# wenbowen123/iros20-6d-pose-tracking

Hardware: NVIDIA H100
Metric: rgbd_pair_frames_per_sec (higher is better)
Workload: dtype bf16x3 (bf16 hi/lo split operands, 3 products/MAC, fp32 accumulate)

## Files before the change

iros20-6d-pose-tracking_b200/csrc/conv_common.h:

```cpp
#pragma once
#include <cstdint>
#include <cuda.h>
#include <cuda_runtime.h>

namespace se3tn {

constexpr int kMaxTaps = 9;
constexpr int kBlockM = 128;
constexpr int kChunkBytes = 128;

enum Act : int { ACT_NONE = 0, ACT_RELU = 1, ACT_SELU = 2 };
enum { KIND_S1 = 0, KIND_S2 = 1, KIND_STEM = 2 };

struct Tap {
    int16_t dy, dx;
};

struct ConvGeom {
    int Hin, Win, in_cstride, in_coff;
    int Ho, Wo, stride;
    int cin;
    int cout;
    int groups;
    int num_taps;
// ... 44 lines not shown

constexpr int kTrunkMaxLayers = 6;

struct TrunkParams {
    LayerDesc layer[kTrunkMaxLayers];
    int n_layers;
    int total_units;
    int img_first, n_img;
    int max_batch;
    unsigned* sched;
    const int* img_wid;
    const CUtensorMap* gbmaps;
    const float* const* gbias;
    unsigned long long* trace;
    int ksplit;
    float* partial;
    unsigned* slice_cnt;
};

struct ResidentParams {
    LayerDesc L;
    int img_first, n_img;
    int m_tiles;
    int step_x, step_y, off_x, off_y;
    const int* img_wid;
    const CUtensorMap* gbmaps;
    const float* const* gbias;
    unsigned long long* trace;
};

cudaError_t launch_conv_resident(const ResidentParams& p, int kind, int prec, int num_sms, bool pdl, cudaStream_t stream);
cudaError_t launch_conv_trunk(const TrunkParams& p, int prec, int num_sms, bool pdl, cudaStream_t stream);
constexpr int kSplitMaxImages = 4, kSplitK = 4, kSplitMaxUnits = kSplitMaxImages * 8 * kTrunkMaxLayers;
inline size_t trunk_sched_words(int max_batch) { return 1 + static_cast<size_t>(kTrunkMaxLayers) * max_batch + static_cast<size_t>(kSplitMaxUnits) * 8; }
inline size_t trunk_partial_floats() { return static_cast<size_t>(kSplitMaxUnits) * kSplitK * 128 * 128; }

cudaError_t launch_conv_direct(const ConvGeom& g, const ConvPtrs& p, cudaStream_t stream);

}
```

iros20-6d-pose-tracking_b200/csrc/conv_wgmma.cu:

```cuda
#include "conv_common.h"
#include "ptx.cuh"
#include "storage.cuh"
#include <algorithm>

namespace se3tn {
namespace {

constexpr int kThreads2 = 384;
constexpr int kPoolPitch = 68;
constexpr int kPoolStageBytes = 121 * kPoolPitch * 4;
constexpr int kPoolStageAlloc = (kPoolStageBytes + 1023) & ~1023;
constexpr int kAUnit3 = 19 * 1024;
constexpr int kAUnitStem = 21 * 1024;
constexpr int kWgRowBytes = 64 * kChunkBytes;

template <int KIND> struct KTab;
template <> struct KTab<KIND_S1> {
    static constexpr int NU = 3;
    __host__ __device__ static constexpr int ntaps(int) { return 3; }
    __host__ __device__ static constexpr int wtap(int u, int k) { return k * 3 + u; }
    __host__ __device__ static constexpr int amap(int) { return 0; }
    __host__ __device__ static constexpr int c1(int u) { return u - 1; }
    __host__ __device__ static constexpr int c2(int) { return -1; }
    __host__ __device__ static constexpr int rows(int) { return 11 * 13; }
// ... 300 lines not shown
                    const int pp = v >> 4, c4 = (v & 15) * 4;
                    const int ppy = pp / 5, ppx = pp - ppy * 5;
                    const int oy = ty * 5 + ppy, ox = tx * 5 + ppx;
                    if (oy >= L.Ho || ox >= L.Wo) continue;
                    float4 mx = make_float4(-3.0e38f, -3.0e38f, -3.0e38f, -3.0e38f);
#pragma unroll
                    for (int dy = 0; dy < 3; ++dy)
#pragma unroll
                        for (int dx = 0; dx < 3; ++dx) {
                            const float4 s4 = *reinterpret_cast<const float4*>(stage + ((2 * ppy + dy) * 11 + 2 * ppx + dx) * kPoolPitch + c4);
                            mx.x = fmaxf(mx.x, s4.x); mx.y = fmaxf(mx.y, s4.y); mx.z = fmaxf(mx.z, s4.z); mx.w = fmaxf(mx.w, s4.w);
                        }
                    const float4 b4 = __ldg(reinterpret_cast<const float4*>(bias + c4));
                    const float v4[4] = {selu_fast(mx.x + b4.x), selu_fast(mx.y + b4.y), selu_fast(mx.z + b4.z), selu_fast(mx.w + b4.w)};
                    S::encode(v4).store(L.out + S::addr((static_cast<size_t>(n0) * L.Ho + oy) * L.Wo + ox, L.out_c, L.out_coff + c4));
                }
                if (C::kPoolBufs == 1) asm volatile("bar.sync 1, 256;" ::: "memory");
            }
        }
        if (stamp) { trace_stamp(p.trace, 4); trace_stamp(p.trace, 6); }
    }

    __syncthreads();
    if (threadIdx.x == 0) trace_exit(p.trace);
}

template <int PREC> struct TCfg {
    static constexpr int BN = 128;
    static constexpr int kAcc = BN / 2;
    static constexpr int kAStages = 3;
    static constexpr int kBStages = 6;
    static constexpr int kBTile = BN * kChunkBytes;
    static constexpr int kEpiPitch = 36;
    static constexpr int kEpiWarpBytes = 16 * kEpiPitch * 4 + 64;
    static constexpr int kEpiBytes = 8 * kEpiWarpBytes;
    static constexpr int kSched = 4;
    static constexpr int kSmem = kAStages * kAUnit3 + kBStages * kBTile + ((kEpiBytes + 1023) & ~1023) + 1024 + 512;
    static_assert(kSmem <= 232448, "shared memory budget");
};

struct UnitCoord { int l, img, tx, ty, n_tile, grp, c0, c1, piece, gidx; };
__device__ __forceinline__ void unit_stamp(const TrunkParams& p, int u, int k) {
    if (p.trace && u < 2048) p.trace[256 * 8 + u * 5 + k] = gtimer();
}

__device__ __forceinline__ int unit_layer(const TrunkParams& p, int u) {
    int l = 0;
#pragma unroll
    for (int i = 1; i < kTrunkMaxLayers; ++i) if (i < p.n_layers && u >= p.layer[i].unit_base) l = i;
    return l;
}

__device__ __forceinline__ UnitCoord decode_unit(const TrunkParams& p, int u) {
    UnitCoord c;
    c.l = unit_layer(p, u);
    const LayerDesc& L = p.layer[c.l];
    int local = u - L.unit_base;
    c.piece = 0; c.c0 = 0; c.c1 = L.chunks;
    if (p.ksplit > 1) {
        c.piece = local % p.ksplit; local /= p.ksplit;
        c.c0 = c.piece * L.chunks / p.ksplit; c.c1 = (c.piece + 1) * L.chunks / p.ksplit;
    }
    c.gidx = L.base_unit0 + local;
    const int im = local / L.units_per_image;
    int r = local - im * L.units_per_image;
    c.img = p.img_first + im;
    c.n_tile = r % L.n_tiles; r /= L.n_tiles;
    c.grp = r % L.groups; r /= L.groups;
    c.ty = r / L.tiles_x; c.tx = r - c.ty * L.tiles_x;
    return c;
}

template <int KIND>
__device__ __forceinline__ void trunk_load_unit(const LayerDesc& L, const UnitCoord& c, uint8_t* sA, uint64_t* a_full, uint64_t* a_empty,
                                                int& stage, uint32_t& phase, int n_stages)
{
// ... 3 lines not shown
    for (int ch = c.c0; ch < c.c1; ++ch) {
#pragma unroll
        for (int u = 0; u < KT::NU; ++u) {
            ptx::mbar_wait(&a_empty[stage], phase ^ 1);
            ptx::mbar_arrive_expect_tx(&a_full[stage], static_cast<uint32_t>(KT::rows(u)) * kChunkBytes);
            ptx::tma_load_4d(sA + stage * kAUnit3, &L.amap[KT::amap(u)], &a_full[stage], cbase + ch * 32, ox + KT::c1(u), oy + KT::c2(u), c.img);
            if (++stage == n_stages) { stage = 0; phase ^= 1; }
        }
    }
}

template <int KIND, int PREC>
__device__ __forceinline__ void trunk_load_weights(const LayerDesc& L, const CUtensorMap* bm, const UnitCoord& c, uint8_t* sB,
                                                   uint64_t* b_full, uint64_t* b_empty, int& stage, uint32_t& phase)
{
    using KT = KTab<KIND>;
    using C = TCfg<PREC>;
    const int wrow = c.grp * L.cout + c.n_tile * C::BN;
    for (int ch = c.c0; ch < c.c1; ++ch) {
#pragma unroll
        for (int u = 0; u < KT::NU; ++u) {
#pragma unroll
            for (int k = 0; k < KT::ntaps(u); ++k) {
                ptx::mbar_wait(&b_empty[stage], phase ^ 1);
                ptx::mbar_arrive_expect_tx(&b_full[stage], C::kBTile);
                ptx::tma_load_2d(sB + stage * C::kBTile, bm, &b_full[stage], KT::wtap(u, k) * L.cin_words + ch * 32, wrow);
                if (++stage == C::kBStages) { stage = 0; phase ^= 1; }
            }
        }
    }
}

template <int KIND, int PREC>
__device__ __forceinline__ void trunk_mma_unit(float (&acc)[TCfg<PREC>::kAcc], const Consumer& cs, int chunks, uint8_t* sA, uint8_t* sB,
                                               uint64_t* a_full, uint64_t* a_empty, uint64_t* b_full, uint64_t* b_empty,
                                               int& astage, uint32_t& aphase, int& bstage, uint32_t& bphase,
                                               unsigned long long* trace, bool first_unit, unsigned long long* ustamp)
{
    using KT = KTab<KIND>;
    using C = TCfg<PREC>;
    const bool stamp = threadIdx.x == 128;
    uint32_t fresh = 0;
    int pend_b = -1, pend_a = -1;
    for (int ch = 0; ch < chunks; ++ch) {
#pragma unroll
        for (int u = 0; u < KT::NU; ++u) {
            ptx::mbar_wait(&a_full[astage], aphase);
            if (first_unit && ch == 0 && u == 0 && stamp) trace_stamp(trace, 3);
            if (ustamp && ch == 0 && u == 0 && stamp) *ustamp = gtimer();
            const uint32_t a_unit_lo = desc_lo(sA + astage * kAUnit3 + cs.cg * kWgRowBytes);
#pragma unroll
            for (int k = 0; k < KT::ntaps(u); ++k) {
                ptx::mbar_wait(&b_full[bstage], bphase);
                if (first_unit && ch == 0 && u == 0 && k == 0 && stamp) trace_stamp(trace, 2);
                const uint32_t b_lo = desc_lo(sB + bstage * C::kBTile);
                const uint32_t a_lo = a_unit_lo + k * kRowShift * (kChunkBytes >> 4);
                ptx::wgmma_fence();
                if constexpr (PREC == SE3TN_PREC_TF32) {
#pragma unroll
                    for (int kk = 0; kk < 4; ++kk)
                        ptx::wgmma_tf32_n128(acc, mk_desc(a_lo + 2 * kk), mk_desc(b_lo + 2 * kk), fresh | (kk ? 1u : 0u));
                } else if constexpr (PREC == SE3TN_PREC_BF16X3) {
                    constexpr int AO[6] = {0, 2, 4, 6, 0, 2};
                    constexpr int BO[6] = {0, 2, 0, 2, 4, 6};
#pragma unroll
                    for (int i = 0; i < 6; ++i)
                        ptx::wgmma_bf16_n128(acc, mk_desc(a_lo + AO[i]), mk_desc(b_lo + BO[i]), fresh | (i ? 1u : 0u));
                } else {
#pragma unroll
                    for (int kk = 0; kk < 4; ++kk)
                        ptx::wgmma_bf16_n128(acc, mk_desc(a_lo + 2 * kk), mk_desc(b_lo + 2 * kk), fresh | (kk ? 1u : 0u));
                }
                ptx::wgmma_commit();
                ptx::wgmma_wait<1>();
                if (cs.leader()) {
                    if (pend_b >= 0) ptx::mbar_arrive(&b_empty[pend_b]);
                    if (pend_a >= 0) ptx::mbar_arrive(&a_empty[pend_a]);
                }
                pend_b = bstage;
                pend_a = (k + 1 == KT::ntaps(u)) ? astage : -1;
                fresh = 1u;
                if (++bstage == C::kBStages) { bstage = 0; bphase ^= 1; }
            }
            if (++astage == C::kAStages) { astage = 0; aphase ^= 1; }
        }
    }
    ptx::wgmma_wait<0>();
    ptx::wgmma_reg_fence(acc);
    if (cs.leader()) {
        if (pend_b >= 0) ptx::mbar_arrive(&b_empty[pend_b]);
        if (pend_a >= 0) ptx::mbar_arrive(&a_empty[pend_a]);
    }
}

template <int PREC>
__global__ void __launch_bounds__(kThreads2, 1)
conv_trunk_kernel(const __grid_constant__ TrunkParams p)
{
    using C = TCfg<PREC>;
    constexpr int BN = C::BN;
    extern __shared__ uint8_t smem_raw[];
    uint8_t* smem = reinterpret_cast<uint8_t*>((reinterpret_cast<uintptr_t>(smem_raw) + 1023) & ~uintptr_t(1023));
    uint8_t* sA = smem;
    uint8_t* sB = sA + C::kAStages * kAUnit3;
    uint8_t* sT = sB + C::kBStages * C::kBTile;
    uint64_t* bars = reinterpret_cast<uint64_t*>(sT + ((C::kEpiBytes + 1023) & ~1023));
    uint64_t* a_full = bars;
    uint64_t* a_empty = a_full + C::kAStages;
    uint64_t* b_full = a_empty + C::kAStages;
    uint64_t* b_empty = b_full + C::kBStages;
    uint64_t* sched_full = b_empty + C::kBStages;
    uint64_t* sched_empty = sched_full + C::kSched;
    int* sched_slot = reinterpret_cast<int*>(sched_empty + C::kSched);

    ptx::grid_dep_launch();
    if (threadIdx.x == 0) trace_stamp(p.trace, 0);
    const int warp = threadIdx.x >> 5;
    const int lane = threadIdx.x & 31;
    unsigned* done = p.sched + 1;

    if (threadIdx.x == 0) {
        for (int s = 0; s < C::kAStages; ++s) { ptx::mbar_init(&a_full[s], 1); ptx::mbar_init(&a_empty[s], 2); }
        for (int s = 0; s < C::kBStages; ++s) { ptx::mbar_init(&b_full[s], 1); ptx::mbar_init(&b_empty[s], 2); }
        for (int s = 0; s < C::kSched; ++s) { ptx::mbar_init(&sched_full[s], 1); ptx::mbar_init(&sched_empty[s], 9); }
        ptx::fence_barrier_init();
        ptx::fence_proxy_async();
    }
    __syncthreads();
    if (threadIdx.x == 0) trace_stamp(p.trace, 1);

    int sslot = 0; uint32_t sphase = 0;
    auto next_unit = [&](bool whole_warp) -> int {
        ptx::mbar_wait(&sched_full[sslot], sphase);
        int u = 0;
        if (lane == 0) u = sched_slot[sslot];
        if (whole_warp) u = __shfl_sync(0xffffffffu, u, 0);
        if (lane == 0) ptx::mbar_arrive(&sched_empty[sslot]);
        if (++sslot == C::kSched) { sslot = 0; sphase ^= 1; }
        return u;
    };

    if (warp == 0) {
        if (lane == 0) {
            for (int l = 0; l < p.n_layers; ++l)
                for (int m = 0; m < (p.layer[l].kind == KIND_S2 ? 4 : 1); ++m) ptx::prefetch_tmap(&p.layer[l].amap[m]);
            ptx::grid_dep_wait();
            int stage = 0; uint32_t phase = 0;
            int ps = 0; uint32_t pph = 0;
            const bool dealt = p.ksplit > 1;
            int u = dealt ? static_cast<int>(blockIdx.x) : static_cast<int>(atomicAdd(p.sched, 1u));
            for (;;) {
                ptx::mbar_wait(&sched_empty[ps], pph ^ 1);
                sched_slot[ps] = u;
                ptx::mbar_arrive(&sched_full[ps]);
                if (++ps == C::kSched) { ps = 0; pph ^= 1; }
                if (u >= p.total_units) break;
                const UnitCoord c = decode_unit(p, u);
                const LayerDesc& L = p.layer[c.l];
                if (L.dep_layer >= 0) {
                    const int* flag = reinterpret_cast<const int*>(done + L.dep_layer * p.max_batch + c.img);
                    if (static_cast<unsigned>(ptx::ld_acquire_gpu(flag)) < L.dep_target) {
                        const long long t0 = clock64();
                        while (static_cast<unsigned>(ptx::ld_acquire_gpu(flag)) < L.dep_target) {
                            __nanosleep(64);
                            if (clock64() - t0 > (1ll << 34)) ptx::timeout_trap();
                        }
                    }
                    ptx::fence_proxy_async_all();
                }
                unit_stamp(p, u, 0);
                if (L.kind == KIND_S1) trunk_load_unit<KIND_S1>(L, c, sA, a_full, a_empty, stage, phase, C::kAStages);
                else                   trunk_load_unit<KIND_S2>(L, c, sA, a_full, a_empty, stage, phase, C::kAStages);
                u = dealt ? u + static_cast<int>(gridDim.x) : static_cast<int>(atomicAdd(p.sched, 1u));
            }
        }
    } else if (warp == 1) {
        if (lane == 0) {
            if (!p.img_wid) for (int l = 0; l < p.n_layers; ++l) ptx::prefetch_tmap(&p.layer[l].bmap);
            int stage = 0; uint32_t phase = 0;
            for (;;) {
                const int u = next_unit(false);
                if (u >= p.total_units) break;
                const UnitCoord c = decode_unit(p, u);
                const LayerDesc& L = p.layer[c.l];
                const CUtensorMap* bm = p.img_wid ? p.gbmaps + p.img_wid[c.img] * kLayersPerSet + L.li : &L.bmap;
                if (L.kind == KIND_S1) trunk_load_weights<KIND_S1, PREC>(L, bm, c, sB, b_full, b_empty, stage, phase);
                else                   trunk_load_weights<KIND_S2, PREC>(L, bm, c, sB, b_full, b_empty, stage, phase);
            }
        }
    } else if (warp >= 4) {
        using S = Storage<PREC>;
        using R4 = Raw<PREC, 4>;
        ptx::grid_dep_wait();
        const Consumer cs;
        const int ew = cs.ew;
        float (*stg)[C::kEpiPitch] = reinterpret_cast<float (*)[C::kEpiPitch]>(sT + ew * C::kEpiWarpBytes);
        int* rowtab = reinterpret_cast<int*>(sT + ew * C::kEpiWarpBytes + 16 * C::kEpiPitch * 4);
        const int grp = lane & 7, sub = lane >> 3;
        int astage = 0; uint32_t aphase = 0;
        int bstage = 0; uint32_t bphase = 0;
        int it = 0;
        for (;; ++it) {
            const int u = next_unit(true);
            if (u >= p.total_units) break;
            const UnitCoord c = decode_unit(p, u);
            const LayerDesc& L = p.layer[c.l];
            const int chunks = L.chunks / p.ksplit;
            {
                const int rw = 16 * ew + (lane & 15);
                const int py = rw / 11, px = rw - py * 11;
                const int y = c.ty * 11 + py, x = c.tx * 11 + px;
                const bool valid = (rw < 121) && (y < L.Ho) && (x < L.Wo);
                __syncwarp();
                if (lane < 16) rowtab[lane] = valid ? (c.img * L.Ho + y) * L.Wo + x : -1;
                __syncwarp();
            }
            int pix[4];
#pragma unroll
            for (int k = 0; k < 4; ++k) pix[k] = rowtab[4 * k + sub];

            float acc[C::kAcc];
#pragma unroll
            for (int i = 0; i < C::kAcc; ++i) acc[i] = 0.f;
            unsigned long long* ust = (p.trace && u < 2048) ? p.trace + 256 * 8 + u * 5 + 1 : nullptr;
            if (L.kind == KIND_S1) trunk_mma_unit<KIND_S1, PREC>(acc, cs, chunks, sA, sB, a_full, a_empty, b_full, b_empty, astage, aphase, bstage, bphase, p.trace, it == 0, ust);
            else                   trunk_mma_unit<KIND_S2, PREC>(acc, cs, chunks, sA, sB, a_full, a_empty, b_full, b_empty, astage, aphase, bstage, bphase, p.trace, it == 0, ust);
            if (threadIdx.x == 128) { unit_stamp(p, u, 2); unit_stamp(p, u, 3); if (it == 0) trace_stamp(p.trace, 5); }

            const int ch0 = c.grp * L.cout + c.n_tile * BN;
            const float* bias_base = p.img_wid ? p.gbias[p.img_wid[c.img] * kLayersPerSet + L.li] : L.bias;
            if (L.res && L.dep_layer >= 0) {
                if (lane == 0) (void)ptx::ld_acquire_gpu(reinterpret_cast<const int*>(done + L.dep_layer * p.max_batch + c.img));
                __syncwarp();
            }
            const bool split = p.ksplit > 1;
            auto slice_of = [&](int pc) -> float* {
                return p.partial + ((static_cast<size_t>(c.gidx) * p.ksplit + pc) * 8 + ew) * (16 * BN);
            };
            unsigned own = 0xFu;
            if (split) {
                float4* d4 = reinterpret_cast<float4*>(slice_of(c.piece)) + lane;
#pragma unroll
                for (int q = 0; q < C::kAcc / 4; ++q) d4[q * 32] = make_float4(acc[4 * q], acc[4 * q + 1], acc[4 * q + 2], acc[4 * q + 3]);
                __threadfence();
                __syncwarp();
                if (lane == 0) atomicAdd(p.slice_cnt + c.gidx * 8 + ew, 1u);
                own = 0u;
#pragma unroll
                for (int bi = 0; bi < BN / 32; ++bi)
                    if (bi * p.ksplit / (BN / 32) == c.piece) own |= 1u << bi;
                if (lane == 0) {
                    const int* cnt = reinterpret_cast<const int*>(p.slice_cnt + c.gidx * 8 + ew);
                    const long long t0 = clock64();
                    while (ptx::ld_acquire_gpu(cnt) < p.ksplit) {
                        __nanosleep(32);
                        if (clock64() - t0 > (1ll << 34)) ptx::timeout_trap();
                    }
                }
                __syncwarp();
                __threadfence();
#pragma unroll
                for (int bi = 0; bi < BN / 32; ++bi) {
                    if (!((own >> bi) & 1u)) continue;
#pragma unroll
                    for (int jj = 0; jj < 4; ++jj) {
                        float4 v[kSplitK];
#pragma unroll
                        for (int pc = 0; pc < kSplitK; ++pc)
                            if (pc < p.ksplit) v[pc] = __ldcg(reinterpret_cast<const float4*>(slice_of(pc)) + lane + bi * 128 + jj * 32);
                        float4 a = make_float4(0.f, 0.f, 0.f, 0.f);
#pragma unroll
                        for (int pc = 0; pc < kSplitK; ++pc)
                            if (pc < p.ksplit) { a.x += v[pc].x; a.y += v[pc].y; a.z += v[pc].z; a.w += v[pc].w; }
                        acc[16 * bi + 4 * jj] = a.x; acc[16 * bi + 4 * jj + 1] = a.y; acc[16 * bi + 4 * jj + 2] = a.z; acc[16 * bi + 4 * jj + 3] = a.w;
                    }
                }
            }
#pragma unroll
            for (int bi = 0; bi < BN / 32; ++bi) {
                if (!((own >> bi) & 1u)) continue;
                const int chan = ch0 + 32 * bi;
                const float4 b4 = __ldg(reinterpret_cast<const float4*>(bias_base + chan + grp * 4));
                R4 rr[4];
                if (L.res) {
#pragma unroll
                    for (int k = 0; k < 4; ++k) {
                        rr[k] = R4{};
                        if (pix[k] >= 0) {
                            const uint8_t* rp = L.res + S::addr(pix[k], L.res_c, chan + grp * 4);
#pragma unroll
                            for (int q = 0; q < R4::kPieces; ++q) rr[k].set(q, __ldcg(R4::at(rp, q)));
                        }
                    }
                }
                __syncwarp();
#pragma unroll
                for (int jj = 0; jj < 4; ++jj)
#pragma unroll
                    for (int h = 0; h < 2; ++h)
                        *reinterpret_cast<float2*>(&stg[cs.R + 8 * h][8 * jj + 2 * cs.m]) = make_float2(acc[16 * bi + 4 * jj + 2 * h], acc[16 * bi + 4 * jj + 2 * h + 1]);
                __syncwarp();
                float4 a4[4];
#pragma unroll
                for (int k = 0; k < 4; ++k) {
                    a4[k] = *reinterpret_cast<const float4*>(&stg[4 * k + sub][grp * 4]);
                    a4[k].x += b4.x; a4[k].y += b4.y; a4[k].z += b4.z; a4[k].w += b4.w;
                }
                if (L.res) {
#pragma unroll
                    for (int k = 0; k < 4; ++k) {
                        float r[4];
                        S::decode(rr[k], r);
                        a4[k].x += r[0]; a4[k].y += r[1]; a4[k].z += r[2]; a4[k].w += r[3];
                    }
                }
                float4 psum = make_float4(0.f, 0.f, 0.f, 0.f);
#pragma unroll
                for (int k = 0; k < 4; ++k) {
                    float4 o = a4[k];
                    o.x = act_apply(o.x, L.act); o.y = act_apply(o.y, L.act); o.z = act_apply(o.z, L.act); o.w = act_apply(o.w, L.act);
                    if (pix[k] < 0) continue;
                    if (L.pool_part) { psum.x += o.x; psum.y += o.y; psum.z += o.z; psum.w += o.w; continue; }
                    const float o4[4] = {o.x, o.y, o.z, o.w};
                    S::encode(o4).store(L.out + S::addr(pix[k], L.out_c, L.out_coff + chan + grp * 4));
                }
                if (L.pool_part) {
#pragma unroll
                    for (int off = 8; off <= 16; off <<= 1) {
                        psum.x += __shfl_xor_sync(0xffffffffu, psum.x, off); psum.y += __shfl_xor_sync(0xffffffffu, psum.y, off);
                        psum.z += __shfl_xor_sync(0xffffffffu, psum.z, off); psum.w += __shfl_xor_sync(0xffffffffu, psum.w, off);
                    }
                    if (sub == 0)
                        *reinterpret_cast<float4*>(L.pool_part + (static_cast<size_t>(c.img) * kPoolSlices + ew) * L.out_c + L.out_coff + chan + grp * 4) = psum;
                }
            }
            if (c.l + 1 < p.n_layers) {
                ptx::fence_proxy_async_all();
                __threadfence();
                __syncwarp();
                if (lane == 0) atomicAdd(done + c.l * p.max_batch + c.img, 1u);
            }
            if (threadIdx.x == 128) unit_stamp(p, u, 4);
        }
        if (threadIdx.x == 128) { trace_stamp(p.trace, 4); trace_stamp(p.trace, 6); }
    }

    __syncthreads();
    if (threadIdx.x == 0) trace_exit(p.trace);
}

template <typename K>
cudaError_t set_smem(K kernel, size_t smem, size_t* cache) {
    int dev = 0;
    if (cudaGetDevice(&dev) != cudaSuccess || dev < 0 || dev >= 64) dev = 0;
    if (smem > cache[dev]) {
        cudaError_t e = cudaFuncSetAttribute(kernel, cudaFuncAttributeMaxDynamicSharedMemorySize, static_cast<int>(smem));
        if (e != cudaSuccess) return e;
        cache[dev] = smem;
    }
    return cudaSuccess;
}

template <int KIND, int PREC>
cudaError_t launch_resident_t(const ResidentParams& p, int num_sms, bool pdl, cudaStream_t stream) {
    using C = RCfg<KIND, PREC>;
    const int tiles_per_tap = (C::kStack == 2) ? 1 : p.L.chunks;
    if ((KIND == KIND_STEM ? 7 : 9) * tiles_per_tap > C::kMaxWTiles) return cudaErrorInvalidValue;
    if (C::kStack == 2 && KIND == KIND_S1 && p.L.chunks != 2) return cudaErrorInvalidValue;
    if (p.L.cout != 64 || p.L.groups != 1 || p.L.n_tiles != 1 || p.m_tiles <= 0) return cudaErrorInvalidValue;
    static size_t attr[64] = {};
    cudaError_t e = set_smem(conv_resident_kernel<KIND, PREC>, C::kSmem, attr);
    if (e != cudaSuccess) return e;
    cudaLaunchConfig_t cfg = {};
    cfg.gridDim = dim3(std::min(p.m_tiles, num_sms)); cfg.blockDim = dim3(kThreads2); cfg.dynamicSmemBytes = C::kSmem; cfg.stream = stream;
    cudaLaunchAttribute at[1];
// ... 58 lines not shown
```

iros20-6d-pose-tracking_b200/csrc/ptx.cuh:

```cuda
#pragma once
#include <cstdint>
#include <cuda.h>

namespace ptx {

__device__ __forceinline__ uint32_t smem_u32(const void* p) {
    return static_cast<uint32_t>(__cvta_generic_to_shared(p));
}

__device__ __forceinline__ bool elect_one() {
    uint32_t pred = 0;
    asm volatile(
        "{\n\t.reg .pred P;\n\t"
        "elect.sync _|P, 0xffffffff;\n\t"
        "selp.u32 %0, 1, 0, P;\n\t}\n"
        : "=r"(pred));
    return pred != 0;
}

__device__ __forceinline__ int ld_acquire_gpu(const int* p) {
    int v;
    asm volatile("ld.acquire.gpu.global.s32 %0, [%1];" : "=r"(v) : "l"(p) : "memory");
    return v;
}
__device__ __forceinline__ void st_release_gpu(int* p, int v) {
    asm volatile("st.release.gpu.global.s32 [%0], %1;" :: "l"(p), "r"(v) : "memory");
}
__device__ __forceinline__ void grid_dep_launch() { asm volatile("griddepcontrol.launch_dependents;" ::: "memory"); }
__device__ __forceinline__ void grid_dep_wait()   { asm volatile("griddepcontrol.wait;" ::: "memory"); }

__device__ __forceinline__ void mbar_init(uint64_t* bar, uint32_t count) {
    asm volatile("mbarrier.init.shared::cta.b64 [%0], %1;" ::"r"(smem_u32(bar)), "r"(count));
}
__device__ __forceinline__ void fence_barrier_init() {
    asm volatile("fence.mbarrier_init.release.cluster;" ::: "memory");
}
__device__ __forceinline__ void fence_proxy_async() {
    asm volatile("fence.proxy.async.shared::cta;" ::: "memory");
}
__device__ __forceinline__ void fence_proxy_async_all() {
    asm volatile("fence.proxy.async;" ::: "memory");
}
__device__ __forceinline__ void mbar_arrive_expect_tx(uint64_t* bar, uint32_t bytes) {
    asm volatile("mbarrier.arrive.expect_tx.shared::cta.b64 _, [%0], %1;"
                 ::"r"(smem_u32(bar)), "r"(bytes) : "memory");
}
__device__ __forceinline__ void mbar_arrive(uint64_t* bar) {
    asm volatile("mbarrier.arrive.shared::cta.b64 _, [%0];" ::"r"(smem_u32(bar)) : "memory");
}
__device__ __forceinline__ bool mbar_try_wait(uint64_t* bar, uint32_t parity) {
    uint32_t ok;
    asm volatile(
        "{\n\t.reg .pred P;\n\t"
        "mbarrier.try_wait.parity.shared::cta.b64 P, [%1], %2;\n\t"
        "selp.u32 %0, 1, 0, P;\n\t}\n"
        : "=r"(ok) : "r"(smem_u32(bar)), "r"(parity) : "memory");
    return ok != 0;
}
static __device__ __noinline__ void timeout_trap() { __trap(); }

__device__ __forceinline__ void mbar_wait(uint64_t* bar, uint32_t parity) {
    if (mbar_try_wait(bar, parity)) return;
// ... 117 lines not shown
```

iros20-6d-pose-tracking_b200/csrc/se3tn.cu:

```cuda
#include "../../include/se3tn.h"
#include "conv_common.h"
#include "aux_kernels.h"
#include "metrics.h"
#include "render.h"
#include <dlfcn.h>
#include "depth_fill.h"
#include "storage.cuh"

#include <algorithm>
#include <cmath>
#include <cstdio>
#include <cstdlib>
#include <cstring>
#include <map>
#include <memory>
#include <string>
#include <type_traits>
#include <vector>

using namespace se3tn;

namespace {

enum Buf { B_X0A, B_X0B, B_Y1A, B_Y1B, B_P1A, B_P1B, B_T1, B_T2, B_U, B_CAT, B_F1, B_T4, B_F2, B_H1, B_H2, B_H3, B_COUNT };
// ... 434 lines not shown
        ++c->launches;
        if (out_feature) { CU_TRY(c, launch_nhwc_to_nchw(bufp(B_F2), out_feature, n, 22 * 22, 256, precision, s)); ++c->launches; }
        return SE3TN_OK;
    }
    if (img_wid) { int rc = sync_tables(c, s); if (rc) return rc; }
    const CUtensorMap* gbmaps = img_wid ? c->d_bmaps[precision].get() : nullptr;
    const float* const* gbias = img_wid ? c->d_bias.get() : nullptr;
    if (c->sched_dirty) { CU_TRY(c, cudaMemsetAsync(c->sched.get(), 0, trunk_sched_words(c->max_batch) * sizeof(unsigned), s)); c->sched_dirty = false; }
    for (int li = 0; li < kFirstTrunkLayer; ++li) {
        ResidentParams rp;
        fill_layer_desc(c, w, li, precision, rp.L);
        rp.img_first = first; rp.n_img = n;
        rp.m_tiles = n * rp.L.tiles_x * rp.L.tiles_y;
        if (kLayers[li].kind == K_STEM) { rp.step_x = rp.step_y = 10; rp.off_x = rp.off_y = -1; }
        else { rp.step_x = rp.step_y = 11; rp.off_x = rp.off_y = 0; }
        rp.img_wid = img_wid; rp.gbmaps = gbmaps; rp.gbias = gbias;
        rp.trace = c->trace ? c->trace.get() + static_cast<size_t>(li) * 256 * 8 : nullptr;
        { ProfScope ps(c, li, s); CU_TRY(c, launch_conv_resident(rp, rp.L.kind, precision, c->num_sms, c->pdl != 0, s)); }
        ++c->launches;
    }
    {
        TrunkParams tp;
        memset(&tp, 0, sizeof tp);
        int ksplit = (n <= kSplitMaxImages) ? kSplitK : 1;
        for (int l = 0; l < 14 - kFirstTrunkLayer; ++l) {
            fill_layer_desc(c, w, kFirstTrunkLayer + l, precision, tp.layer[l]);
            while (tp.layer[l].chunks % ksplit) ksplit /= 2;
        }
        int base = 0, base0 = 0;
        for (int l = 0; l < 14 - kFirstTrunkLayer; ++l) {
            LayerDesc& d = tp.layer[l];
            d.unit_base = base; base += n * d.units_per_image * ksplit;
            d.base_unit0 = base0; base0 += n * d.units_per_image;
            if (l > 0) { d.dep_layer = l - 1; d.dep_target = 8u * static_cast<unsigned>(ksplit) * static_cast<unsigned>(tp.layer[l - 1].units_per_image); }
        }
        if (ksplit > 1 && base0 > kSplitMaxUnits) return fail(c, SE3TN_ERR_STATE, "split-K scratch too small");
        tp.ksplit = ksplit; tp.partial = c->partial.get();
        tp.slice_cnt = c->sched.get() + 1 + static_cast<size_t>(kTrunkMaxLayers) * c->max_batch;
        tp.layer[5].pool_part = c->pool_part.get();
        tp.n_layers = 6; tp.total_units = base;
        tp.img_first = first; tp.n_img = n; tp.max_batch = c->max_batch;
        tp.sched = c->sched.get(); tp.img_wid = img_wid; tp.gbmaps = gbmaps; tp.gbias = gbias;
        tp.trace = c->trace ? c->trace.get() + static_cast<size_t>(kFirstTrunkLayer) * 256 * 8 : nullptr;
        c->sched_dirty = true;
        { ProfScope ps(c, kFirstTrunkLayer, s); CU_TRY(c, launch_conv_trunk(tp, precision, c->num_sms, c->pdl != 0, s)); }
        ++c->launches;
    }
    {
        ProfScope ps(c, 16, s);
        CU_TRY(c, launch_head_pooled(c->pool_part.get() + static_cast<size_t>(first) * kPoolSlices * 1024, fcw, fcw + 6 * 512, out_trans, out_rot, n, 121,
                                     img_wid ? img_wid + first : nullptr, img_wid ? c->d_fc.get() : nullptr,
                                     pose ? pose->in : nullptr, pose ? pose->out : nullptr, pose ? pose->tn : 0.f, pose ? pose->rn : 0.f,
                                     c->sched.get(), static_cast<int>(trunk_sched_words(c->max_batch)), s));
        c->sched_dirty = false;
        if (pose && pose_done) *pose_done = true;
    }
    ++c->launches;
    if (out_feature) { CU_TRY(c, launch_nhwc_to_nchw(reinterpret_cast<const uint8_t*>(c->buf[B_F2]) + static_cast<size_t>(first) * 22 * 22 * 256 * prec_bytes_per_channel(precision), out_feature, n, 22 * 22, 256,
                                                       precision, s)); ++c->launches; }
    return SE3TN_OK;
}

int prepare_weights(se3tn_ctx* c, DeviceWeights& w, const float* blob) {
    const size_t floats = blob_floats();
    CU_TRY(c, dev_alloc(w.blob, floats));
    for (int p : kTensorPrecs) CU_TRY(c, dev_alloc(w.conv[p], floats * prec_bytes_per_channel(p)));
    CU_TRY(c, dev_alloc(w.stack, 8 * 128 * 288 * sizeof(float)));
// ... 759 lines not shown
```

Before: 26730.

## Ping-pong consumer warpgroups over whole tiles with register reallocation

Each consumer warpgroup now takes whole 128-row units in alternation and computes both 64-row halves into two accumulator sets. A named-barrier turn token orders their MMA phases, so one group's epilogue overlaps the other's MMA. Producer warps give up registers through setmaxnreg and consumers gain them to hold the doubled accumulators. Barrier arrival counts, dependency targets and per-slice counters are halved to match one consumer per unit. This risks register pressure and spills, and the ring-skip bookkeeping must stay exactly in step with the producers.

Result: faster. 28050, median of 6 (+4.9%).

```diff
diff --git a/iros20-6d-pose-tracking_b200/csrc/conv_common.h b/iros20-6d-pose-tracking_b200/csrc/conv_common.h
--- a/iros20-6d-pose-tracking_b200/csrc/conv_common.h
+++ b/iros20-6d-pose-tracking_b200/csrc/conv_common.h
@@ -100,7 +100,7 @@
 cudaError_t launch_conv_resident(const ResidentParams& p, int kind, int prec, int num_sms, bool pdl, cudaStream_t stream);
 cudaError_t launch_conv_trunk(const TrunkParams& p, int prec, int num_sms, bool pdl, cudaStream_t stream);
 constexpr int kSplitMaxImages = 4, kSplitK = 4, kSplitMaxUnits = kSplitMaxImages * 8 * kTrunkMaxLayers;
-inline size_t trunk_sched_words(int max_batch) { return 1 + static_cast<size_t>(kTrunkMaxLayers) * max_batch + static_cast<size_t>(kSplitMaxUnits) * 8; }
+inline size_t trunk_sched_words(int max_batch) { return 1 + static_cast<size_t>(kTrunkMaxLayers) * max_batch + static_cast<size_t>(kSplitMaxUnits) * 4; }
 inline size_t trunk_partial_floats() { return static_cast<size_t>(kSplitMaxUnits) * kSplitK * 128 * 128; }
 
 cudaError_t launch_conv_direct(const ConvGeom& g, const ConvPtrs& p, cudaStream_t stream);
diff --git a/iros20-6d-pose-tracking_b200/csrc/conv_wgmma.cu b/iros20-6d-pose-tracking_b200/csrc/conv_wgmma.cu
--- a/iros20-6d-pose-tracking_b200/csrc/conv_wgmma.cu
+++ b/iros20-6d-pose-tracking_b200/csrc/conv_wgmma.cu
@@ -356,16 +356,26 @@
     static constexpr int kBStages = 6;
     static constexpr int kBTile = BN * kChunkBytes;
     static constexpr int kEpiPitch = 36;
-    static constexpr int kEpiWarpBytes = 16 * kEpiPitch * 4 + 64;
+    static constexpr int kEpiWarpBytes = 16 * kEpiPitch * 4 + 128;
     static constexpr int kEpiBytes = 8 * kEpiWarpBytes;
     static constexpr int kSched = 4;
     static constexpr int kSmem = kAStages * kAUnit3 + kBStages * kBTile + ((kEpiBytes + 1023) & ~1023) + 1024 + 512;
     static_assert(kSmem <= 232448, "shared memory budget");
 };
+constexpr int kProducerRegs = 40;
+constexpr int kConsumerRegs = 232;
+constexpr int kTurnBar = 1;
+constexpr int kTaps3 = 9;
+
+__device__ __forceinline__ void ring_skip(int& stage, uint32_t& phase, int n, int stages) {
+    stage += n;
+    phase ^= static_cast<uint32_t>(stage / stages) & 1u;
+    stage %= stages;
+}
 
 struct UnitCoord { int l, img, tx, ty, n_tile, grp, c0, c1, piece, gidx; };
 __device__ __forceinline__ void unit_stamp(const TrunkParams& p, int u, int k) {
-    if (p.trace && u < 2048) p.trace[256 * 8 + u * 5 + k] = gtimer();
+    if (p.trace && u < 2048) p.trace[256 * 8 + u * 5 + k] = k == 4 ? (gtimer() & ~0xffull) | (blockIdx.x & 0xff) : gtimer();
 }
 
 __device__ __forceinline__ int unit_layer(const TrunkParams& p, int u) {
@@ -435,44 +445,48 @@
 }
 
 template <int KIND, int PREC>
-__device__ __forceinline__ void trunk_mma_unit(float (&acc)[TCfg<PREC>::kAcc], const Consumer& cs, int chunks, uint8_t* sA, uint8_t* sB,
+__device__ __forceinline__ void trunk_mma_unit(float (&acc)[2][TCfg<PREC>::kAcc], const Consumer& cs, int chunks, uint8_t* sA, uint8_t* sB,
                                                uint64_t* a_full, uint64_t* a_empty, uint64_t* b_full, uint64_t* b_empty,
                                                int& astage, uint32_t& aphase, int& bstage, uint32_t& bphase,
                                                unsigned long long* trace, bool first_unit, unsigned long long* ustamp)
 {
     using KT = KTab<KIND>;
     using C = TCfg<PREC>;
-    const bool stamp = threadIdx.x == 128;
+    const bool stamp = cs.leader();
     uint32_t fresh = 0;
     int pend_b = -1, pend_a = -1;
+    ptx::bar_sync(kTurnBar + cs.cg, 256);
     for (int ch = 0; ch < chunks; ++ch) {
 #pragma unroll
         for (int u = 0; u < KT::NU; ++u) {
             ptx::mbar_wait(&a_full[astage], aphase);
             if (first_unit && ch == 0 && u == 0 && stamp) trace_stamp(trace, 3);
             if (ustamp && ch == 0 && u == 0 && stamp) *ustamp = gtimer();
-            const uint32_t a_unit_lo = desc_lo(sA + astage * kAUnit3 + cs.cg * kWgRowBytes);
+            const uint32_t a_unit_lo = desc_lo(sA + astage * kAUnit3);
 #pragma unroll
             for (int k = 0; k < KT::ntaps(u); ++k) {
                 ptx::mbar_wait(&b_full[bstage], bphase);
                 if (first_unit && ch == 0 && u == 0 && k == 0 && stamp) trace_stamp(trace, 2);
                 const uint32_t b_lo = desc_lo(sB + bstage * C::kBTile);
-                const uint32_t a_lo = a_unit_lo + k * kRowShift * (kChunkBytes >> 4);
                 ptx::wgmma_fence();
-                if constexpr (PREC == SE3TN_PREC_TF32) {
-#pragma unroll
-                    for (int kk = 0; kk < 4; ++kk)
-                        ptx::wgmma_tf32_n128(acc, mk_desc(a_lo + 2 * kk), mk_desc(b_lo + 2 * kk), fresh | (kk ? 1u : 0u));
-                } else if constexpr (PREC == SE3TN_PREC_BF16X3) {
-                    constexpr int AO[6] = {0, 2, 4, 6, 0, 2};
-                    constexpr int BO[6] = {0, 2, 0, 2, 4, 6};
-#pragma unroll
-                    for (int i = 0; i < 6; ++i)
-                        ptx::wgmma_bf16_n128(acc, mk_desc(a_lo + AO[i]), mk_desc(b_lo + BO[i]), fresh | (i ? 1u : 0u));
-                } else {
-#pragma unroll
-                    for (int kk = 0; kk < 4; ++kk)
-                        ptx::wgmma_bf16_n128(acc, mk_desc(a_lo + 2 * kk), mk_desc(b_lo + 2 * kk), fresh | (kk ? 1u : 0u));
+#pragma unroll
+                for (int hf = 0; hf < 2; ++hf) {
+                    const uint32_t a_lo = a_unit_lo + hf * (kWgRowBytes >> 4) + k * kRowShift * (kChunkBytes >> 4);
+                    if constexpr (PREC == SE3TN_PREC_TF32) {
+#pragma unroll
+                        for (int kk = 0; kk < 4; ++kk)
+                            ptx::wgmma_tf32_n128(acc[hf], mk_desc(a_lo + 2 * kk), mk_desc(b_lo + 2 * kk), fresh | (kk ? 1u : 0u));
+                    } else if constexpr (PREC == SE3TN_PREC_BF16X3) {
+                        constexpr int AO[6] = {0, 2, 4, 6, 0, 2};
+                        constexpr int BO[6] = {0, 2, 0, 2, 4, 6};
+#pragma unroll
+                        for (int i = 0; i < 6; ++i)
+                            ptx::wgmma_bf16_n128(acc[hf], mk_desc(a_lo + AO[i]), mk_desc(b_lo + BO[i]), fresh | (i ? 1u : 0u));
+                    } else {
+#pragma unroll
+                        for (int kk = 0; kk < 4; ++kk)
+                            ptx::wgmma_bf16_n128(acc[hf], mk_desc(a_lo + 2 * kk), mk_desc(b_lo + 2 * kk), fresh | (kk ? 1u : 0u));
+                    }
                 }
                 ptx::wgmma_commit();
                 ptx::wgmma_wait<1>();
@@ -488,8 +502,10 @@
             if (++astage == C::kAStages) { astage = 0; aphase ^= 1; }
         }
     }
+    ptx::bar_arrive(kTurnBar + (cs.cg ^ 1), 256);
     ptx::wgmma_wait<0>();
-    ptx::wgmma_reg_fence(acc);
+    ptx::wgmma_reg_fence(acc[0]);
+    ptx::wgmma_reg_fence(acc[1]);
     if (cs.leader()) {
         if (pend_b >= 0) ptx::mbar_arrive(&b_empty[pend_b]);
         if (pend_a >= 0) ptx::mbar_arrive(&a_empty[pend_a]);
@@ -523,8 +539,8 @@
     unsigned* done = p.sched + 1;
 
     if (threadIdx.x == 0) {
-        for (int s = 0; s < C::kAStages; ++s) { ptx::mbar_init(&a_full[s], 1); ptx::mbar_init(&a_empty[s], 2); }
-        for (int s = 0; s < C::kBStages; ++s) { ptx::mbar_init(&b_full[s], 1); ptx::mbar_init(&b_empty[s], 2); }
+        for (int s = 0; s < C::kAStages; ++s) { ptx::mbar_init(&a_full[s], 1); ptx::mbar_init(&a_empty[s], 1); }
+        for (int s = 0; s < C::kBStages; ++s) { ptx::mbar_init(&b_full[s], 1); ptx::mbar_init(&b_empty[s], 1); }
         for (int s = 0; s < C::kSched; ++s) { ptx::mbar_init(&sched_full[s], 1); ptx::mbar_init(&sched_empty[s], 9); }
         ptx::fence_barrier_init();
         ptx::fence_proxy_async();
@@ -543,117 +559,138 @@
         return u;
     };
 
-    if (warp == 0) {
-        if (lane == 0) {
-            for (int l = 0; l < p.n_layers; ++l)
-                for (int m = 0; m < (p.layer[l].kind == KIND_S2 ? 4 : 1); ++m) ptx::prefetch_tmap(&p.layer[l].amap[m]);
-            ptx::grid_dep_wait();
-            int stage = 0; uint32_t phase = 0;
-            int ps = 0; uint32_t pph = 0;
-            const bool dealt = p.ksplit > 1;
-            int u = dealt ? static_cast<int>(blockIdx.x) : static_cast<int>(atomicAdd(p.sched, 1u));
-            for (;;) {
-                ptx::mbar_wait(&sched_empty[ps], pph ^ 1);
-                sched_slot[ps] = u;
-                ptx::mbar_arrive(&sched_full[ps]);
-                if (++ps == C::kSched) { ps = 0; pph ^= 1; }
-                if (u >= p.total_units) break;
-                const UnitCoord c = decode_unit(p, u);
-                const LayerDesc& L = p.layer[c.l];
-                if (L.dep_layer >= 0) {
-                    const int* flag = reinterpret_cast<const int*>(done + L.dep_layer * p.max_batch + c.img);
-                    if (static_cast<unsigned>(ptx::ld_acquire_gpu(flag)) < L.dep_target) {
-                        const long long t0 = clock64();
-                        while (static_cast<unsigned>(ptx::ld_acquire_gpu(flag)) < L.dep_target) {
-                            __nanosleep(64);
-                            if (clock64() - t0 > (1ll << 34)) ptx::timeout_trap();
+    if (warp < 4) {
+        ptx::setmaxnreg_dec<kProducerRegs>();
+        if (warp == 0) {
+            if (lane == 0) {
+                for (int l = 0; l < p.n_layers; ++l)
+                    for (int m = 0; m < (p.layer[l].kind == KIND_S2 ? 4 : 1); ++m) ptx::prefetch_tmap(&p.layer[l].amap[m]);
+                ptx::grid_dep_wait();
+                int stage = 0; uint32_t phase = 0;
+                int ps = 0; uint32_t pph = 0;
+                const bool dealt = p.ksplit > 1;
+                int u = dealt ? static_cast<int>(blockIdx.x) : static_cast<int>(atomicAdd(p.sched, 1u));
+                for (;;) {
+                    ptx::mbar_wait(&sched_empty[ps], pph ^ 1);
+                    sched_slot[ps] = u;
+                    ptx::mbar_arrive(&sched_full[ps]);
+                    if (++ps == C::kSched) { ps = 0; pph ^= 1; }
+                    if (u >= p.total_units) break;
+                    const UnitCoord c = decode_unit(p, u);
+                    const LayerDesc& L = p.layer[c.l];
+                    if (L.dep_layer >= 0) {
+                        const int* flag = reinterpret_cast<const int*>(done + L.dep_layer * p.max_batch + c.img);
+                        if (static_cast<unsigned>(ptx::ld_acquire_gpu(flag)) < L.dep_target) {
+                            const long long t0 = clock64();
+                            while (static_cast<unsigned>(ptx::ld_acquire_gpu(flag)) < L.dep_target) {
+                                __nanosleep(64);
+                                if (clock64() - t0 > (1ll << 34)) ptx::timeout_trap();
+                            }
                         }
-                    }
-                    ptx::fence_proxy_async_all();
-                }
-                unit_stamp(p, u, 0);
-                if (L.kind == KIND_S1) trunk_load_unit<KIND_S1>(L, c, sA, a_full, a_empty, stage, phase, C::kAStages);
-                else                   trunk_load_unit<KIND_S2>(L, c, sA, a_full, a_empty, stage, phase, C::kAStages);
-                u = dealt ? u + static_cast<int>(gridDim.x) : static_cast<int>(atomicAdd(p.sched, 1u));
-            }
-        }
-    } else if (warp == 1) {
-        if (lane == 0) {
-            if (!p.img_wid) for (int l = 0; l < p.n_layers; ++l) ptx::prefetch_tmap(&p.layer[l].bmap);
-            int stage = 0; uint32_t phase = 0;
-            for (;;) {
-                const int u = next_unit(false);
-                if (u >= p.total_units) break;
-                const UnitCoord c = decode_unit(p, u);
-                const LayerDesc& L = p.layer[c.l];
-                const CUtensorMap* bm = p.img_wid ? p.gbmaps + p.img_wid[c.img] * kLayersPerSet + L.li : &L.bmap;
-                if (L.kind == KIND_S1) trunk_load_weights<KIND_S1, PREC>(L, bm, c, sB, b_full, b_empty, stage, phase);
-                else                   trunk_load_weights<KIND_S2, PREC>(L, bm, c, sB, b_full, b_empty, stage, phase);
-            }
-        }
-    } else if (warp >= 4) {
+                        ptx::fence_proxy_async_all();
+                    }
+                    unit_stamp(p, u, 0);
+                    if (L.kind == KIND_S1) trunk_load_unit<KIND_S1>(L, c, sA, a_full, a_empty, stage, phase, C::kAStages);
+                    else                   trunk_load_unit<KIND_S2>(L, c, sA, a_full, a_empty, stage, phase, C::kAStages);
+                    u = dealt ? u + static_cast<int>(gridDim.x) : static_cast<int>(atomicAdd(p.sched, 1u));
+                }
+            }
+        } else if (warp == 1) {
+            if (lane == 0) {
+                if (!p.img_wid) for (int l = 0; l < p.n_layers; ++l) ptx::prefetch_tmap(&p.layer[l].bmap);
+                int stage = 0; uint32_t phase = 0;
+                for (;;) {
+                    const int u = next_unit(false);
+                    if (u >= p.total_units) break;
+                    const UnitCoord c = decode_unit(p, u);
+                    const LayerDesc& L = p.layer[c.l];
+                    const CUtensorMap* bm = p.img_wid ? p.gbmaps + p.img_wid[c.img] * kLayersPerSet + L.li : &L.bmap;
+                    if (L.kind == KIND_S1) trunk_load_weights<KIND_S1, PREC>(L, bm, c, sB, b_full, b_empty, stage, phase);
+                    else                   trunk_load_weights<KIND_S2, PREC>(L, bm, c, sB, b_full, b_empty, stage, phase);
+                }
+            }
+        }
+    } else {
+        ptx::setmaxnreg_inc<kConsumerRegs>();
         using S = Storage<PREC>;
         using R4 = Raw<PREC, 4>;
         ptx::grid_dep_wait();
         const Consumer cs;
-        const int ew = cs.ew;
-        float (*stg)[C::kEpiPitch] = reinterpret_cast<float (*)[C::kEpiPitch]>(sT + ew * C::kEpiWarpBytes);
-        int* rowtab = reinterpret_cast<int*>(sT + ew * C::kEpiWarpBytes + 16 * C::kEpiPitch * 4);
+        const int cw = cs.cw;
+        float (*stg)[C::kEpiPitch] = reinterpret_cast<float (*)[C::kEpiPitch]>(sT + cs.ew * C::kEpiWarpBytes);
+        int* rowtab = reinterpret_cast<int*>(sT + cs.ew * C::kEpiWarpBytes + 16 * C::kEpiPitch * 4);
         const int grp = lane & 7, sub = lane >> 3;
         int astage = 0; uint32_t aphase = 0;
         int bstage = 0; uint32_t bphase = 0;
-        int it = 0;
-        for (;; ++it) {
+        if (cs.cg == 1) ptx::bar_arrive(kTurnBar, 256);
+        for (int it = 0;; ++it) {
             const int u = next_unit(true);
-            if (u >= p.total_units) break;
+            const bool mine = (it & 1) == cs.cg;
+            if (u >= p.total_units) {
+                if (mine) ptx::bar_sync(kTurnBar + cs.cg, 256);
+                break;
+            }
             const UnitCoord c = decode_unit(p, u);
             const LayerDesc& L = p.layer[c.l];
             const int chunks = L.chunks / p.ksplit;
+            if (!mine) {
+                ring_skip(astage, aphase, chunks * (L.kind == KIND_S1 ? KTab<KIND_S1>::NU : KTab<KIND_S2>::NU), C::kAStages);
+                ring_skip(bstage, bphase, chunks * kTaps3, C::kBStages);
+                continue;
+            }
             {
-                const int rw = 16 * ew + (lane & 15);
+                const int rw = 64 * (lane >> 4) + 16 * cw + (lane & 15);
                 const int py = rw / 11, px = rw - py * 11;
                 const int y = c.ty * 11 + py, x = c.tx * 11 + px;
                 const bool valid = (rw < 121) && (y < L.Ho) && (x < L.Wo);
                 __syncwarp();
-                if (lane < 16) rowtab[lane] = valid ? (c.img * L.Ho + y) * L.Wo + x : -1;
+                rowtab[lane] = valid ? (c.img * L.Ho + y) * L.Wo + x : -1;
                 __syncwarp();
             }
-            int pix[4];
-#pragma unroll
-            for (int k = 0; k < 4; ++k) pix[k] = rowtab[4 * k + sub];
-
-            float acc[C::kAcc];
-#pragma unroll
-            for (int i = 0; i < C::kAcc; ++i) acc[i] = 0.f;
+            const int ch0 = c.grp * L.cout + c.n_tile * BN;
+            const float* bias_base = p.img_wid ? p.gbias[p.img_wid[c.img] * kLayersPerSet + L.li] : L.bias;
+            float4 b4[BN / 32];
+#pragma unroll
+            for (int bi = 0; bi < BN / 32; ++bi) b4[bi] = __ldg(reinterpret_cast<const float4*>(bias_base + ch0 + 32 * bi + grp * 4));
+
+            float acc[2][C::kAcc];
+#pragma unroll
+            for (int i = 0; i < C::kAcc; ++i) { acc[0][i] = 0.f; acc[1][i] = 0.f; }
             unsigned long long* ust = (p.trace && u < 2048) ? p.trace + 256 * 8 + u * 5 + 1 : nullptr;
             if (L.kind == KIND_S1) trunk_mma_unit<KIND_S1, PREC>(acc, cs, chunks, sA, sB, a_full, a_empty, b_full, b_empty, astage, aphase, bstage, bphase, p.trace, it == 0, ust);
             else                   trunk_mma_unit<KIND_S2, PREC>(acc, cs, chunks, sA, sB, a_full, a_empty, b_full, b_empty, astage, aphase, bstage, bphase, p.trace, it == 0, ust);
-            if (threadIdx.x == 128) { unit_stamp(p, u, 2); unit_stamp(p, u, 3); if (it == 0) trace_stamp(p.trace, 5); }
-
-            const int ch0 = c.grp * L.cout + c.n_tile * BN;
-            const float* bias_base = p.img_wid ? p.gbias[p.img_wid[c.img] * kLayersPerSet + L.li] : L.bias;
+            if (cs.leader()) { unit_stamp(p, u, 2); unit_stamp(p, u, 3); if (it == 0) trace_stamp(p.trace, 5); }
+            int pix[2][4];
+#pragma unroll
+            for (int hf = 0; hf < 2; ++hf)
+#pragma unroll
+                for (int k = 0; k < 4; ++k) pix[hf][k] = rowtab[16 * hf + 4 * k + sub];
+
             if (L.res && L.dep_layer >= 0) {
                 if (lane == 0) (void)ptx::ld_acquire_gpu(reinterpret_cast<const int*>(done + L.dep_layer * p.max_batch + c.img));
                 __syncwarp();
             }
             const bool split = p.ksplit > 1;
             auto slice_of = [&](int pc) -> float* {
-                return p.partial + ((static_cast<size_t>(c.gidx) * p.ksplit + pc) * 8 + ew) * (16 * BN);
+                return p.partial + ((static_cast<size_t>(c.gidx) * p.ksplit + pc) * 4 + cw) * (32 * BN);
             };
             unsigned own = 0xFu;
             if (split) {
                 float4* d4 = reinterpret_cast<float4*>(slice_of(c.piece)) + lane;
 #pragma unroll
-                for (int q = 0; q < C::kAcc / 4; ++q) d4[q * 32] = make_float4(acc[4 * q], acc[4 * q + 1], acc[4 * q + 2], acc[4 * q + 3]);
+                for (int hf = 0; hf < 2; ++hf)
+#pragma unroll
+                    for (int q = 0; q < C::kAcc / 4; ++q)
+                        d4[(hf * C::kAcc / 4 + q) * 32] = make_float4(acc[hf][4 * q], acc[hf][4 * q + 1], acc[hf][4 * q + 2], acc[hf][4 * q + 3]);
                 __threadfence();
                 __syncwarp();
-                if (lane == 0) atomicAdd(p.slice_cnt + c.gidx * 8 + ew, 1u);
+                if (lane == 0) atomicAdd(p.slice_cnt + c.gidx * 4 + cw, 1u);
                 own = 0u;
 #pragma unroll
                 for (int bi = 0; bi < BN / 32; ++bi)
                     if (bi * p.ksplit / (BN / 32) == c.piece) own |= 1u << bi;
                 if (lane == 0) {
-                    const int* cnt = reinterpret_cast<const int*>(p.slice_cnt + c.gidx * 8 + ew);
+                    const int* cnt = reinterpret_cast<const int*>(p.slice_cnt + c.gidx * 4 + cw);
                     const long long t0 = clock64();
                     while (ptx::ld_acquire_gpu(cnt) < p.ksplit) {
                         __nanosleep(32);
@@ -663,78 +700,83 @@
                 __syncwarp();
                 __threadfence();
 #pragma unroll
+                for (int hf = 0; hf < 2; ++hf)
+#pragma unroll
+                    for (int bi = 0; bi < BN / 32; ++bi) {
+                        if (!((own >> bi) & 1u)) continue;
+#pragma unroll
+                        for (int jj = 0; jj < 4; ++jj) {
+                            float4 v[kSplitK];
+#pragma unroll
+                            for (int pc = 0; pc < kSplitK; ++pc)
+                                if (pc < p.ksplit) v[pc] = __ldcg(reinterpret_cast<const float4*>(slice_of(pc)) + lane + (hf * C::kAcc / 4 + 4 * bi + jj) * 32);
+                            float4 a = make_float4(0.f, 0.f, 0.f, 0.f);
+#pragma unroll
+                            for (int pc = 0; pc < kSplitK; ++pc)
+                                if (pc < p.ksplit) { a.x += v[pc].x; a.y += v[pc].y; a.z += v[pc].z; a.w += v[pc].w; }
+                            acc[hf][16 * bi + 4 * jj] = a.x; acc[hf][16 * bi + 4 * jj + 1] = a.y; acc[hf][16 * bi + 4 * jj + 2] = a.z; acc[hf][16 * bi + 4 * jj + 3] = a.w;
+                        }
+                    }
+            }
+#pragma unroll
+            for (int hf = 0; hf < 2; ++hf) {
+                const int slice = 4 * hf + cw;
+#pragma unroll
                 for (int bi = 0; bi < BN / 32; ++bi) {
                     if (!((own >> bi) & 1u)) continue;
-#pragma unroll
-                    for (int jj = 0; jj < 4; ++jj) {
-                        float4 v[kSplitK];
-#pragma unroll
-                        for (int pc = 0; pc < kSplitK; ++pc)
-                            if (pc < p.ksplit) v[pc] = __ldcg(reinterpret_cast<const float4*>(slice_of(pc)) + lane + bi * 128 + jj * 32);
-                        float4 a = make_float4(0.f, 0.f, 0.f, 0.f);
-#pragma unroll
-                        for (int pc = 0; pc < kSplitK; ++pc)
-                            if (pc < p.ksplit) { a.x += v[pc].x; a.y += v[pc].y; a.z += v[pc].z; a.w += v[pc].w; }
-                        acc[16 * bi + 4 * jj] = a.x; acc[16 * bi + 4 * jj + 1] = a.y; acc[16 * bi + 4 * jj + 2] = a.z; acc[16 * bi + 4 * jj + 3] = a.w;
-                    }
-                }
-            }
-#pragma unroll
-            for (int bi = 0; bi < BN / 32; ++bi) {
-                if (!((own >> bi) & 1u)) continue;
-                const int chan = ch0 + 32 * bi;
-                const float4 b4 = __ldg(reinterpret_cast<const float4*>(bias_base + chan + grp * 4));
-                R4 rr[4];
-                if (L.res) {
+                    const int chan = ch0 + 32 * bi;
+                    R4 rr[4];
+                    if (L.res) {
+#pragma unroll
+                        for (int k = 0; k < 4; ++k) {
+                            rr[k] = R4{};
+                            if (pix[hf][k] >= 0) {
+                                const uint8_t* rp = L.res + S::addr(pix[hf][k], L.res_c, chan + grp * 4);
+#pragma unroll
+                                for (int q = 0; q < R4::kPieces; ++q) rr[k].set(q, __ldcg(R4::at(rp, q)));
+                            }
+                        }
+                    }
+                    __syncwarp();
+#pragma unroll
+                    for (int jj = 0; jj < 4; ++jj)
+#pragma unroll
+                        for (int h = 0; h < 2; ++h)
+                            *reinterpret_cast<float2*>(&stg[cs.R + 8 * h][8 * jj + 2 * cs.m]) = make_float2(acc[hf][16 * bi + 4 * jj + 2 * h], acc[hf][16 * bi + 4 * jj + 2 * h + 1]);
+                    __syncwarp();
+                    float4 a4[4];
 #pragma unroll
                     for (int k = 0; k < 4; ++k) {
-                        rr[k] = R4{};
-                        if (pix[k] >= 0) {
-                            const uint8_t* rp = L.res + S::addr(pix[k], L.res_c, chan + grp * 4);
-#pragma unroll
-                            for (int q = 0; q < R4::kPieces; ++q) rr[k].set(q, __ldcg(R4::at(rp, q)));
+                        a4[k] = *reinterpret_cast<const float4*>(&stg[4 * k + sub][grp * 4]);
+                        a4[k].x += b4[bi].x; a4[k].y += b4[bi].y; a4[k].z += b4[bi].z; a4[k].w += b4[bi].w;
+                    }
+                    if (L.res) {
+#pragma unroll
+                        for (int k = 0; k < 4; ++k) {
+                            float r[4];
+                            S::decode(rr[k], r);
+                            a4[k].x += r[0]; a4[k].y += r[1]; a4[k].z += r[2]; a4[k].w += r[3];
                         }
                     }
-                }
-                __syncwarp();
-#pragma unroll
-                for (int jj = 0; jj < 4; ++jj)
-#pragma unroll
-                    for (int h = 0; h < 2; ++h)
-                        *reinterpret_cast<float2*>(&stg[cs.R + 8 * h][8 * jj + 2 * cs.m]) = make_float2(acc[16 * bi + 4 * jj + 2 * h], acc[16 * bi + 4 * jj + 2 * h + 1]);
-                __syncwarp();
-                float4 a4[4];
-#pragma unroll
-                for (int k = 0; k < 4; ++k) {
-                    a4[k] = *reinterpret_cast<const float4*>(&stg[4 * k + sub][grp * 4]);
-                    a4[k].x += b4.x; a4[k].y += b4.y; a4[k].z += b4.z; a4[k].w += b4.w;
-                }
-                if (L.res) {
+                    float4 psum = make_float4(0.f, 0.f, 0.f, 0.f);
 #pragma unroll
                     for (int k = 0; k < 4; ++k) {
-                        float r[4];
-                        S::decode(rr[k], r);
-                        a4[k].x += r[0]; a4[k].y += r[1]; a4[k].z += r[2]; a4[k].w += r[3];
-                    }
-                }
-                float4 psum = make_float4(0.f, 0.f, 0.f, 0.f);
-#pragma unroll
-                for (int k = 0; k < 4; ++k) {
-                    float4 o = a4[k];
-                    o.x = act_apply(o.x, L.act); o.y = act_apply(o.y, L.act); o.z = act_apply(o.z, L.act); o.w = act_apply(o.w, L.act);
-                    if (pix[k] < 0) continue;
-                    if (L.pool_part) { psum.x += o.x; psum.y += o.y; psum.z += o.z; psum.w += o.w; continue; }
-                    const float o4[4] = {o.x, o.y, o.z, o.w};
-                    S::encode(o4).store(L.out + S::addr(pix[k], L.out_c, L.out_coff + chan + grp * 4));
-                }
-                if (L.pool_part) {
-#pragma unroll
-                    for (int off = 8; off <= 16; off <<= 1) {
-                        psum.x += __shfl_xor_sync(0xffffffffu, psum.x, off); psum.y += __shfl_xor_sync(0xffffffffu, psum.y, off);
-                        psum.z += __shfl_xor_sync(0xffffffffu, psum.z, off); psum.w += __shfl_xor_sync(0xffffffffu, psum.w, off);
-                    }
-                    if (sub == 0)
-                        *reinterpret_cast<float4*>(L.pool_part + (static_cast<size_t>(c.img) * kPoolSlices + ew) * L.out_c + L.out_coff + chan + grp * 4) = psum;
+                        float4 o = a4[k];
+                        o.x = act_apply(o.x, L.act); o.y = act_apply(o.y, L.act); o.z = act_apply(o.z, L.act); o.w = act_apply(o.w, L.act);
+                        if (pix[hf][k] < 0) continue;
+                        if (L.pool_part) { psum.x += o.x; psum.y += o.y; psum.z += o.z; psum.w += o.w; continue; }
+                        const float o4[4] = {o.x, o.y, o.z, o.w};
+                        S::encode(o4).store(L.out + S::addr(pix[hf][k], L.out_c, L.out_coff + chan + grp * 4));
+                    }
+                    if (L.pool_part) {
+#pragma unroll
+                        for (int off = 8; off <= 16; off <<= 1) {
+                            psum.x += __shfl_xor_sync(0xffffffffu, psum.x, off); psum.y += __shfl_xor_sync(0xffffffffu, psum.y, off);
+                            psum.z += __shfl_xor_sync(0xffffffffu, psum.z, off); psum.w += __shfl_xor_sync(0xffffffffu, psum.w, off);
+                        }
+                        if (sub == 0)
+                            *reinterpret_cast<float4*>(L.pool_part + (static_cast<size_t>(c.img) * kPoolSlices + slice) * L.out_c + L.out_coff + chan + grp * 4) = psum;
+                    }
                 }
             }
             if (c.l + 1 < p.n_layers) {
@@ -743,7 +785,7 @@
                 __syncwarp();
                 if (lane == 0) atomicAdd(done + c.l * p.max_batch + c.img, 1u);
             }
-            if (threadIdx.x == 128) unit_stamp(p, u, 4);
+            if (cs.leader()) unit_stamp(p, u, 4);
         }
         if (threadIdx.x == 128) { trace_stamp(p.trace, 4); trace_stamp(p.trace, 6); }
     }
diff --git a/iros20-6d-pose-tracking_b200/csrc/ptx.cuh b/iros20-6d-pose-tracking_b200/csrc/ptx.cuh
--- a/iros20-6d-pose-tracking_b200/csrc/ptx.cuh
+++ b/iros20-6d-pose-tracking_b200/csrc/ptx.cuh
@@ -28,6 +28,11 @@
 }
 __device__ __forceinline__ void grid_dep_launch() { asm volatile("griddepcontrol.launch_dependents;" ::: "memory"); }
 __device__ __forceinline__ void grid_dep_wait()   { asm volatile("griddepcontrol.wait;" ::: "memory"); }
+
+template <int N> __device__ __forceinline__ void setmaxnreg_dec() { asm volatile("setmaxnreg.dec.sync.aligned.u32 %0;" ::"n"(N)); }
+template <int N> __device__ __forceinline__ void setmaxnreg_inc() { asm volatile("setmaxnreg.inc.sync.aligned.u32 %0;" ::"n"(N)); }
+__device__ __forceinline__ void bar_sync(int id, int n)   { asm volatile("bar.sync %0, %1;" ::"r"(id), "r"(n) : "memory"); }
+__device__ __forceinline__ void bar_arrive(int id, int n) { asm volatile("bar.arrive %0, %1;" ::"r"(id), "r"(n) : "memory"); }
 
 __device__ __forceinline__ void mbar_init(uint64_t* bar, uint32_t count) {
     asm volatile("mbarrier.init.shared::cta.b64 [%0], %1;" ::"r"(smem_u32(bar)), "r"(count));
diff --git a/iros20-6d-pose-tracking_b200/csrc/se3tn.cu b/iros20-6d-pose-tracking_b200/csrc/se3tn.cu
--- a/iros20-6d-pose-tracking_b200/csrc/se3tn.cu
+++ b/iros20-6d-pose-tracking_b200/csrc/se3tn.cu
@@ -490,7 +490,7 @@
             LayerDesc& d = tp.layer[l];
             d.unit_base = base; base += n * d.units_per_image * ksplit;
             d.base_unit0 = base0; base0 += n * d.units_per_image;
-            if (l > 0) { d.dep_layer = l - 1; d.dep_target = 8u * static_cast<unsigned>(ksplit) * static_cast<unsigned>(tp.layer[l - 1].units_per_image); }
+            if (l > 0) { d.dep_layer = l - 1; d.dep_target = 4u * static_cast<unsigned>(ksplit) * static_cast<unsigned>(tp.layer[l - 1].units_per_image); }
         }
         if (ksplit > 1 && base0 > kSplitMaxUnits) return fail(c, SE3TN_ERR_STATE, "split-K scratch too small");
         tp.ksplit = ksplit; tp.partial = c->partial.get();
```
